# RustAudio/lewton

Hardware: NVIDIA H100
Metric: Msamples/s IMDCT+window+OLA, 2048-pt long blocks (higher is better)
Workload: dtype f32

## Files before the change

### lewton_b200/build.py

```python
import os
import re
import shutil
import subprocess

HERE = os.path.dirname(os.path.abspath(__file__))
CSRC = os.path.join(HERE, "csrc")
SO = os.path.join(HERE, "liblewton_b200.so")
K_LONG_REGS = 249
SOURCES = ["lwb_api.cu", "host_objects.cuh", "path_generic.cuh", "path_long.cuh", "path_chain.cuh", "path_mixed.cuh", "path_mid.cuh",
           "tables_host.cpp", "frontend.cpp", "batcher_submit.cpp", "batcher.h", "lwb_common.h", "pcm_copy_plan.h", "kernels_generic.cuh", "kernel_long.cuh", "kernel_deal.cuh", "kernel_short.cuh", "kernel_mid.cuh", "kernel_chain.cuh", "kernel_prologue.cuh", "kernel_floor0.cuh", "floor1_eval.cuh",
           "floor1_inverse_db.inc", "Makefile"]


def _stale():
    if not os.path.exists(SO):
        return True
    t = os.path.getmtime(SO)
    deps = [os.path.join(CSRC, s) for s in SOURCES] + [os.path.join(HERE, "..", "include", h)
                                                       for h in ("lewton_b200.h", "lewton_frontend.h")]
    return any(os.path.getmtime(d) > t for d in deps)


def check_no_fma(so=SO):
    if shutil.which("cuobjdump") is None:
# ... 41 lines not shown
```

### lewton_b200/csrc/host_objects.cuh

```cuda
#pragma once

struct DevBuf {
    void *p = nullptr;
    size_t cap = 0;
};

struct Staging {
    void *h = nullptr;
    size_t cap = 0;
    cudaEvent_t ev = nullptr;
    bool pending = false;
};

struct ArenaSet {
    DevBuf coeffs, dense, pcm, kinds, ys, vqoff, vqrec;
    cudaEvent_t done = nullptr;
};
constexpr int kHostSets = 2;

struct CachedTables {
    DevTables dt;
    std::vector<float> a, b, c, w;
    std::vector<uint32_t> br;
    std::vector<void *> allocs;
// ... 6 lines not shown
    cudaStream_t copy_in = nullptr, copy_out = nullptr;
    cudaEvent_t ev_in[64] = {}, ev_done[65] = {};
    DevBuf runs_buf[2];
    cudaEvent_t ev_desc[2] = {}, ev_kdone[2] = {};
    int runs_par = 0;
    uint32_t ticket_next = 0;
    uint64_t epoch = 0;
    uint64_t state_gen = 1;
    std::string err;
    uint64_t launches = 0;
    uint64_t kernel_launches[LWB_KERNEL_COUNT] = {};
    std::vector<PcmSpan> pcm_spans;
    std::vector<PcmCopy> pcm_copies;
    std::deque<CachedTables> tables;
    DevBuf spec, segtab, magic, x, desc, chains, ticket, cdesc, cbytes;
    DevBuf floor0;
    ArenaSet host_sets[kHostSets];
    int host_next = 0;
    ArenaSet ordered;
    Staging stage[3];
    int stage_next = 0;
    std::vector<void *> stage_old;
    uint64_t tickets_issued = 0, tickets_done = 0;
    std::deque<cudaEvent_t> ticket_events;
    std::vector<cudaEvent_t> spare_events;
    size_t x_cap_elems = (size_t)64 << 20;
};

struct lwb_setup {
    lwb_ctx *ctx = nullptr;
    DevSetup host;
    DevSetup *d_setup = nullptr;
    std::vector<void *> allocs;
    uint8_t channels = 0, bs0 = 0, bs1 = 0;
    uint32_t n_modes = 0;
    uint32_t n_mappings = 0;
    std::vector<DevMapping> mappings;
    std::vector<uint8_t> floor_types;
    std::vector<DevFloor0> floor0;
    mutable bool streams_opened = false;
    bool floor0_described(uint32_t fi) const { return fi < floor0.size() && floor0[fi].order != 0; }
    unsigned out_channels() const { return host.n_out ? host.n_out : channels; }
};

struct RowCopy { const float *src; float *dst; uint32_t n4, pad; };
struct ChainShape { unsigned warps; size_t smem; int n1max, wpc, np; };

struct Step {
    int kernel;
    const void *desc;
    size_t n;
    const float *pack;
};

struct StepArgs {
    void *pcm = nullptr;
    int out_format = LWB_OUT_F32_PLANAR;
    const float *w_short = nullptr;
    int ls = 0;
    int mid_kb = 0;
// ... 28 lines not shown
    lwb_batch_io io;
    bool captured = false;
    uint64_t gen = 0;
    FrontStages front;
    DevBuf pro, mix;
    StepArgs args;
    std::vector<Step> steps;
};

struct lwb_stream {
    lwb_ctx *ctx = nullptr;
    const lwb_setup *setup = nullptr;
    float *d_state = nullptr;
    bool has = false;
    uint32_t plen = 0;
    uint64_t busy_epoch = 0;
};

static void capture(lwb_plan *plan, uint64_t gen, const FrontStages &front, const StepArgs &args, std::vector<Step> steps)
{
    plan->captured = true;
    plan->gen = gen;
    plan->front = front;
    for (size_t i = 0; i < plan->n_chains && front.n; i++)
        if (!plan->chains[i].stream->setup->floor0.empty()) plan->front.floor0 = true;
    plan->args = args;
    plan->steps = std::move(steps);
}


static inline void set_stream_state(lwb_stream *s, bool has, uint32_t plen)
{
    if (s->has != has || s->plen != plen) {
        s->has = has;
        s->plen = plen;
        s->ctx->state_gen++;
    }
}

static int fail(lwb_ctx *ctx, int code, const char *what, cudaError_t e = cudaSuccess)
{
    if (ctx) {
        ctx->err = what;
        if (e != cudaSuccess) {
            ctx->err += ": ";
            ctx->err += cudaGetErrorString(e);
        }
    }
    return code;
}
// ... 190 lines not shown
```

### lewton_b200/csrc/kernel_long.cuh

```cuda
#pragma once
#include <stdint.h>

#include "lwb_common.h"

#if defined(__CUDACC__)
#include <cuda_fp16.h>
#include <cuda_runtime.h>

#include <type_traits>
#define LWB_HD __host__ __device__ __forceinline__
#else
#define LWB_HD inline
#endif

namespace lwb {

constexpr int kLongBs = 11;
constexpr int kLongN = 2048;
constexpr int kLongN2 = 1024;

struct alignas(16) LongRun {
    const float *in;
    void *out;
    float *state;
    uint32_t in_stride;
    uint32_t n_packets;
    uint8_t has_prev;
    uint8_t write_state;
    uint8_t dummy;
    uint8_t first_short;
    uint8_t last_short;
    uint8_t pad[3];
    float *state_out;
};
static_assert(sizeof(LongRun) == 48, "LongRun is copied by TMA in 16-byte units");

struct V { float x, y; };

#if defined(__CUDA_ARCH__)
__device__ __forceinline__ V vadd(V a, V b) { return V{__fadd_rn(a.x, b.x), __fadd_rn(a.y, b.y)}; }
__device__ __forceinline__ V vsub(V a, V b) { return V{__fsub_rn(a.x, b.x), __fsub_rn(a.y, b.y)}; }
__device__ __forceinline__ V vmul(V a, V b) { return V{__fmul_rn(a.x, b.x), __fmul_rn(a.y, b.y)}; }
__device__ __forceinline__ V vadd_p(V a, V b) { return V{__fadd_rn(a.x, b.x), __fadd_rn(a.y, b.y)}; }
__device__ __forceinline__ V vsub_p(V a, V b) { return V{__fsub_rn(a.x, b.x), __fsub_rn(a.y, b.y)}; }
__device__ __forceinline__ V vnsub_p(V a, V b) { return V{__fsub_rn(-a.x, b.x), __fsub_rn(-a.y, b.y)}; }
#else
inline V vadd(V a, V b) { return V{a.x + b.x, a.y + b.y}; }
// ... 403 lines not shown
#define LWB_KA(j) (4u * (uint32_t)swz(64 * (j)))
#define LWB_KB(j, h) (4u * (uint32_t)swz(((h) << 6) | ((j) << 3)))
#define LWB_KC(j) (4u * (uint32_t)swz(j))

struct RunCur {
    const float *in;
    void *out;
    float *state;
    uint32_t in_stride;
    uint32_t flags;
};
__device__ __forceinline__ RunCur run_cur(const LongRun &r)
{
    return RunCur{r.in, r.out, r.state, r.in_stride,
                  (uint32_t)(r.has_prev ? 1u : 0u) | (r.write_state ? 2u : 0u) | (r.dummy ? 4u : 0u) |
                      (r.first_short ? 8u : 0u) | (r.last_short ? 16u : 0u)};
}
struct RunCurS : RunCur { float *state_out; };
__device__ __forceinline__ RunCurS run_cur_s(const LongRun &r)
{
    RunCurS c;
    static_cast<RunCur &>(c) = run_cur(r);
    c.flags |= r.first_short == 2 ? 32u : 0u;
    c.state_out = r.state_out ? r.state_out : r.state;
    return c;
}

__device__ __forceinline__ int16_t d_sample_i16(float v)
{
    short r;
    asm("cvt.rzi.s16.f32 %0, %1;" : "=h"(r) : "f"(__fmul_rn(v, 32768.0f)));
// ... 12 lines not shown
__device__ __forceinline__ void st_pcm(int16_t *p, float v) { __stcs(reinterpret_cast<short *>(p), (short)d_sample_i16(v)); }
__device__ __forceinline__ void st_pcm(__half *p, float v) { __stcs(reinterpret_cast<short *>(p), __half_as_short(d_sample_f16(v))); }

template <SampleKind K>
using sample_t = std::conditional_t<K == kSampleF32, float, std::conditional_t<K == kSampleI16, int16_t, __half>>;

template <int FORMAT>
__device__ __forceinline__ void store_sample(void *pcm, uint64_t off, uint64_t stride, unsigned channels, unsigned ch,
                                             uint64_t i, float v)
{
    constexpr OutFormat F = out_format_of(FORMAT);
    using T = sample_t<F.kind>;
    static_cast<T *>(pcm)[off + (F.planar ? (uint64_t)ch * stride + i : i * channels + ch)] = d_sample(v, static_cast<T *>(nullptr));
}

template <int NB, bool FIRST, typename OutT, typename RC = RunCur>
__device__ __forceinline__ void out_stage(const TwMix &tw, int lane, const V O[NB][8], const V E[NB][8], V pe[NB][8],
                                          const RC cur[NB], OutT *out[NB], const float *s_state)
{
#pragma unroll
    for (int j = 0; j < 8; j++) {
        const int r64 = 64 * rev3(j);
        const bool nat = (j & 1);
        const V b0 = tw(P_B0 + j), b1 = tw(P_B1 + j);
        const V wlo = tw(P_WLO + j), whi = tw(P_WHI + j);
#pragma unroll
        for (int b = 0; b < NB; b++) {
            V plo = pe[b][j], phi = pe[b][j];
            bool emit = !(cur[b].flags & 4u);
            if (FIRST) {
                emit = emit && (cur[b].flags & 1u);
                if (cur[b].flags & 1u) {
                    const float *s_lo = s_state + b * kLongN2 + lane, *s_hi = s_state + b * kLongN2 + 63 - lane;
                    const float ax = nat ? s_lo[r64] : s_hi[r64], ay = nat ? s_hi[r64] : s_lo[r64];
                    const float bx = nat ? s_hi[960 - r64] : s_lo[960 - r64];
                    const float by = nat ? s_lo[960 - r64] : s_hi[960 - r64];
                    plo = V{ax, ay};
                    phi = V{bx, by};
                }
            }
            V lo, hi, pev;
            step8_ola(b0, b1, wlo, whi, O[b][j], E[b][j], plo, phi, lo, hi, pev);
            pe[b][j] = pev;
            if (emit) {
                OutT *o_lo = out[b] + lane, *o_hi = out[b] + 63 - lane;
                if (nat) {
                    st_pcm(o_lo + r64, lo.x); st_pcm(o_hi + r64, lo.y);
                    st_pcm(o_hi + 960 - r64, hi.x); st_pcm(o_lo + 960 - r64, hi.y);
                } else {
                    st_pcm(o_hi + r64, lo.x); st_pcm(o_lo + r64, lo.y);
                    st_pcm(o_lo + 960 - r64, hi.x); st_pcm(o_hi + 960 - r64, hi.y);
                }
            }
// ... 113 lines not shown
        const uint32_t bar = bars_s + 8 * stage;
        mbar_expect_tx(bar, kLongStageBytes);
#pragma unroll
        for (int b = 0; b < NB; b++)
            tma_load_1d(tiles_s + stage * kLongStageBytes + b * kLongTileBytes,
                        r[b].in + (size_t)pkt * r[b].in_stride, kLongTileBytes, bar);
    };
    auto issue_stage_cur = [&](uint32_t stage, uint32_t pkt) {
        const uint32_t bar = bars_s + 8 * stage;
        mbar_expect_tx(bar, kLongStageBytes);
#pragma unroll
        for (int b = 0; b < NB; b++)
            tma_load_1d(tiles_s + stage * kLongStageBytes + b * kLongTileBytes,
                        cur[b].in + (size_t)pkt * cur[b].in_stride, kLongTileBytes, bar);
    };
    auto issue_state = [&](const float *const st[NB], const uint32_t has[NB]) {
        uint32_t bytes = 0;
#pragma unroll
        for (int b = 0; b < NB; b++) bytes += has[b] ? kLongTileBytes : 0;
        mbar_expect_tx(bar_state, bytes);
#pragma unroll
        for (int b = 0; b < NB; b++)
            if (has[b]) tma_load_1d(state_s + b * kLongTileBytes, st[b], kLongTileBytes, bar_state);
    };

    {
        uint32_t idx = 0;
        if (lane == 0) idx = atomicAdd(ticket, 1u);
        idx = __shfl_sync(0xffffffffu, idx, 0);
        if (idx >= n_groups) return;
#pragma unroll
        for (int b = 0; b < NB; b++) cur[b] = run_cur(runs[idx * NB + b]);
        npk = runs[idx * NB].n_packets;
        if (lane == 0) {
            fence_proxy_async();
            const float *st[NB];
            uint32_t has[NB];
#pragma unroll
            for (int b = 0; b < NB; b++) { st[b] = cur[b].state; has[b] = cur[b].flags & 1u; }
            issue_state(st, has);
            for (; lc < (uint32_t)kLongRing && lc < npk; lc++) issue_stage_cur(lc, lc);
            nx_idx = atomicAdd(ticket, 1u);
        }
    }

    for (;;) {
        V pe[NB][8];
#pragma unroll
        for (int b = 0; b < NB; b++)
#pragma unroll
            for (int j = 0; j < 8; j++) pe[b][j] = V{0.f, 0.f};
        OutT *out[NB];
#pragma unroll
        for (int b = 0; b < NB; b++) out[b] = static_cast<OutT *>(cur[b].out);

// ... 85 lines not shown
                            issue_stage(tgt, s_next, nx_lc);
                            nx_lc++;
                        }
                    }
                }
            }
            phase_c_fft<NB>(tw, O, E);
            if (p > 0) {
                out_stage<NB, false, OutT>(tw, lane, O, E, pe, cur, out, s_state);
            } else {
                mbar_wait(bar_state, (phase_bits >> 30) & 1u);
                phase_bits ^= 1u << 30;
                if (NB == 1 && (cur[0].flags & 8u))
                    out_first_short<NB, OutT>(tw, lane, O, E, pe, cur, out, s_state, w_short, ls);
                else
                    out_stage<NB, true, OutT>(tw, lane, O, E, pe, cur, out, s_state);
                __syncwarp();
            }
#pragma unroll
            for (int b = 0; b < NB; b++)
                if (p > 0 || (cur[b].flags & 1u)) out[b] += (p == 0 && (cur[b].flags & 8u)) ? kLongN2 - ls : kLongN2;
            if (lane == 0 && nx_stage == 2 && !nx_state_issued) {
                const float *st[NB];
                uint32_t has[NB];
#pragma unroll
                for (int b = 0; b < NB; b++) { st[b] = s_next[b].state; has[b] = s_next[b].has_prev; }
                fence_proxy_async();
                issue_state(st, has);
                nx_state_issued = 1;
            }
            slot_i = (slot_i + 1 == (uint32_t)kLongRing) ? 0 : slot_i + 1;
        }
#pragma unroll
        for (int b = 0; b < NB; b++) {
            if ((cur[b].flags & 16u)) {
                const bool emitted = (npk > 1 || (cur[b].flags & 1u)) && !(cur[b].flags & 4u);
                const bool keep = (cur[b].flags & 6u) == 2u;
#pragma unroll
                for (int j = 0; j < 8; j++) {
                    const int r64 = 64 * rev3(j);
#pragma unroll
                    for (int h = 0; h < 2; h++) {
                        const float v = ((j & 1) != 0) == (h == 0) ? pe[b][j].x : pe[b][j].y;
// ... 1 lines not shown
                        if (m < ls) {
                            if (emitted) st_pcm(out[b] + m, v);
                        } else if (keep && m < kLongN2 - ls) {
                            cur[b].state[m - ls] = v;
                            cur[b].state[kLongN2 - 1 - ls - m] = v;
                        }
                    }
                }
            } else if ((cur[b].flags & 6u) == 2u) {
                float *s_lo = cur[b].state + lane, *s_hi = cur[b].state + 63 - lane;
#pragma unroll
                for (int j = 0; j < 8; j++) {
                    const int r64 = 64 * rev3(j);
                    const float vx = (j & 1) ? pe[b][j].x : pe[b][j].y, vy = (j & 1) ? pe[b][j].y : pe[b][j].x;
                    s_lo[r64] = vx; s_hi[r64] = vy;
                    s_hi[960 - r64] = vx; s_lo[960 - r64] = vy;
                }
            }
        }
        uint32_t st_ = 0, nlc = 0;
        if (lane == 0) {
            if (nx_stage == 0) {
                if (nx_idx < n_groups) {
                    fence_proxy_async();
                    mbar_expect_tx(bar_desc, NB * (uint32_t)sizeof(LongRun));
                    tma_load_1d(next_s, runs + (size_t)nx_idx * NB, NB * (uint32_t)sizeof(LongRun), bar_desc);
                    nx_stage = 1;
                } else {
                    nx_stage = 3;
                }
            }
            if (nx_stage == 1) {
                mbar_wait(bar_desc, desc_parity);
                desc_parity ^= 1u;
                nx_stage = 2;
                nx_npk = s_next[0].n_packets;
                nx_lc = 0;
            }
            if (nx_stage == 2 && !nx_state_issued) {
                const float *st[NB];
                uint32_t has[NB];
#pragma unroll
                for (int b = 0; b < NB; b++) { st[b] = s_next[b].state; has[b] = s_next[b].has_prev; }
                fence_proxy_async();
                issue_state(st, has);
            }
            st_ = nx_stage;
            nlc = nx_lc;
        }
        st_ = __shfl_sync(0xffffffffu, st_, 0);
        nlc = __shfl_sync(0xffffffffu, nlc, 0);
        if (st_ != 2) break;
        __syncwarp();
#pragma unroll
        for (int b = 0; b < NB; b++) cur[b] = run_cur(s_next[b]);
        npk = s_next[0].n_packets;
        __syncwarp();
        lc = nlc;
        nx_stage = 0; nx_lc = 0; nx_npk = 0; nx_state_issued = 0;
        if (lane == 0) {
// ... 244 lines not shown
```

### lewton_b200/csrc/lwb_api.cu

```cuda
#include <cuda_runtime.h>
#include <sched.h>
#include <sys/syscall.h>
#include <unistd.h>

#include <algorithm>
#include <cctype>
#include <cmath>
#include <cstdio>
#include <cstdlib>
#include <cstring>
#include <deque>
#include <new>
#include <string>
#include <vector>

#include "kernel_long.cuh"
#include "kernel_short.cuh"
#include "kernel_mid.cuh"
#include "kernels_generic.cuh"
#include "kernel_chain.cuh"
#include "kernel_prologue.cuh"
#include "kernel_floor0.cuh"
#include "lwb_common.h"
#include "pcm_copy_plan.h"
// ... 65 lines not shown
{
    cudaError_t e = cudaStreamSynchronize(ctx->stream);
    for (cudaStream_t s : {ctx->copy_in, ctx->copy_out}) {
        const cudaError_t e2 = s ? cudaStreamSynchronize(s) : cudaSuccess;
        if (e == cudaSuccess) e = e2;
    }
    return e;
}

extern "C" void lwb_ctx_destroy(lwb_ctx *ctx)
{
    if (!ctx) return;
    cudaSetDevice(ctx->device);
    sync_all_streams(ctx);
    for (DevBuf *b : {&ctx->spec, &ctx->segtab, &ctx->magic, &ctx->x, &ctx->desc, &ctx->chains, &ctx->ticket, &ctx->runs_buf[0],
                      &ctx->runs_buf[1], &ctx->cdesc, &ctx->cbytes, &ctx->floor0})
        if (b->p) cudaFree(b->p);
    auto free_set = [](ArenaSet &s) {
        for (DevBuf *b : {&s.coeffs, &s.dense, &s.pcm, &s.kinds, &s.ys, &s.vqoff, &s.vqrec})
            if (b->p) cudaFree(b->p);
        if (s.done) cudaEventDestroy(s.done);
    };
    for (ArenaSet &s : ctx->host_sets) free_set(s);
    free_set(ctx->ordered);
    for (cudaEvent_t e : ctx->ticket_events) cudaEventDestroy(e);
    for (cudaEvent_t e : ctx->spare_events) cudaEventDestroy(e);
    for (CachedTables &ct : ctx->tables)
        for (void *p : ct.allocs) cudaFree(p);
    for (void *h : ctx->stage_old) cudaFreeHost(h);
    for (Staging &st : ctx->stage) {
        if (st.h) cudaFreeHost(st.h);
// ... 432 lines not shown
}

extern "C" void lwb_stream_destroy(lwb_stream *s)
{
    if (!s) return;
    cudaSetDevice(s->ctx->device);
    sync_all_streams(s->ctx);
    cudaFree(s->d_state);
    delete s;
}

extern "C" int lwb_stream_reset(lwb_stream *s)
{
    if (!s) return LWB_ERR_INVALID;
    set_stream_state(s, false, 0);
    return LWB_OK;
}
extern "C" int lwb_stream_is_empty(const lwb_stream *s) { return (!s || !s->has) ? 1 : 0; }
extern "C" uint32_t lwb_stream_state_len(const lwb_stream *s) { return (s && s->has) ? s->plen : 0; }

extern "C" int lwb_stream_clone(const lwb_stream *s, lwb_stream **out)
{
    if (!s || !out) return LWB_ERR_INVALID;
    int rc = lwb_stream_open(s->ctx, s->setup, out);
    if (rc) return rc;
    (*out)->has = s->has;
    (*out)->plen = s->plen;
    lwb_ctx *ctx = s->ctx;
    CU(ctx, cudaMemcpyAsync((*out)->d_state, s->d_state,
                            s->setup->channels * state_stride(s->setup) * sizeof(float),
                            cudaMemcpyDeviceToDevice, ctx->stream));
    return LWB_OK;
}

extern "C" int lwb_stream_export_state(lwb_stream *s, float *out)
{
    if (!s || !out) return LWB_ERR_INVALID;
    if (!s->has) return LWB_OK;
    lwb_ctx *ctx = s->ctx;
    CU(ctx, cudaSetDevice(ctx->device));
    CU(ctx, cudaMemcpy2DAsync(out, s->plen * sizeof(float), s->d_state, state_stride(s->setup) * sizeof(float),
                              s->plen * sizeof(float), s->setup->channels, cudaMemcpyDeviceToHost, ctx->stream));
    CU(ctx, cudaStreamSynchronize(ctx->stream));
    return LWB_OK;
}

extern "C" int lwb_stream_import_state(lwb_stream *s, const float *data, uint32_t len)
{
    if (!s || (!data && len)) return LWB_ERR_INVALID;
    if (len > state_stride(s->setup)) return LWB_ERR_BUFFER;
    lwb_ctx *ctx = s->ctx;
    CU(ctx, cudaSetDevice(ctx->device));
    if (len) {
        CU(ctx, cudaMemcpy2DAsync(s->d_state, state_stride(s->setup) * sizeof(float), data, len * sizeof(float),
                                  len * sizeof(float), s->setup->channels, cudaMemcpyHostToDevice, ctx->stream));
        CU(ctx, cudaStreamSynchronize(ctx->stream));
    }
    s->ctx->state_gen++;
    s->has = true;
    s->plen = len;
    return LWB_OK;
}

extern "C" int lwb_decoded_sample_count(const lwb_setup *su, uint8_t mode, int prev_flag, int next_flag,
                                        uint32_t *n_samples)
{
    if (!su || !n_samples) return LWB_ERR_INVALID;
    Geom g;
    int rc = geometry(su, mode, prev_flag, next_flag, &g);
    if (rc) return rc;
    *n_samples = g.rs - g.ls;
    return LWB_OK;
}

#include "path_generic.cuh"
#include "path_long.cuh"
#include "path_chain.cuh"
#include "path_mixed.cuh"
#include "path_mid.cuh"

using BatchPath = int (*)(lwb_ctx *, const lwb_chain *, size_t, const lwb_batch_io *, const BatchWalk &, bool *, lwb_plan *);
static constexpr BatchPath kBatchPaths[] = {try_long, try_mid, try_mixed, try_chain, try_generic};
constexpr size_t kChainPath = 3, kGenericPath = 4;
static_assert(kBatchPaths[kChainPath] == try_chain && kBatchPaths[kGenericPath] == try_generic && std::size(kBatchPaths) == kGenericPath + 1,
              "kChainPath / kGenericPath name the chain-kernel and the four-kernel path, the last one");

static size_t first_batch_path()
{
    const char *fg = getenv("LWB_FORCE_GENERIC");
    if (!fg) return 0;
    return std::strcmp(fg, "1") == 0 ? kGenericPath : kChainPath;
}

static int check_batch_args(lwb_ctx *ctx, const lwb_chain *chains, size_t n_chains, const lwb_batch_io *io)
{
    if (io->entry != LWB_ENTRY_SPECTRUM && io->entry != LWB_ENTRY_RESIDUE && io->entry != LWB_ENTRY_VQ) return fail(ctx, LWB_ERR_INVALID, "bad entry");
    if (io->memory != LWB_MEM_HOST && io->memory != LWB_MEM_DEVICE) return fail(ctx, LWB_ERR_INVALID, "bad memory space");
    if (!out_format_known(io->out_format)) return fail(ctx, LWB_ERR_INVALID, "bad out_format");
    if (n_chains == 0) return LWB_OK;
    if ((!io->coeffs && io->entry != LWB_ENTRY_VQ) || !io->pcm) return fail(ctx, LWB_ERR_INVALID, "null arena");
// ... 25 lines not shown
    for (size_t i = 0; i < n_chains; i++) {
        const lwb_chain *c = &chains[i];
        const ChainWalk &w = bw->walks[i] = walk_chain(c, [](uint32_t, const Geom &, bool, uint32_t, uint64_t, uint64_t) {});
        if (!w.done) continue;
        if (planar && c->out_stride < w.n_samples) return fail(ctx, LWB_ERR_BUFFER, "chain: out_stride smaller than the samples produced");
        ext.add(io, c, w);
        if (io->entry != LWB_ENTRY_SPECTRUM && (rc = scan_floor_kinds(ctx, io, c, w.done, &ext.need_dense, &ext.need_floor0))) return rc;
    }
    if (ext.need_dense && !io->dense_floor) return fail(ctx, LWB_ERR_INVALID, "dense_floor missing");
    if ((rc = check_vq_offsets(ctx, io, ext.r_lo, ext.r_hi))) return rc;
    if (!pinned_only || io->memory != LWB_MEM_HOST || ext.empty()) return LWB_OK;
    CU(ctx, cudaSetDevice(ctx->device));
    return check_page_locked(ctx, io, ext, chains[0].stream->setup->channels);
}

static int queue_batch(lwb_ctx *ctx, lwb_chain *chains, size_t n_chains, const lwb_batch_io *io, lwb_plan *prepared, bool pinned_only)
{
    if (!ctx || (!chains && n_chains) || !io) return LWB_ERR_INVALID;
    BatchWalk bw;
    int rc = walk_batch(ctx, chains, n_chains, io, pinned_only, &bw);
    if (rc || n_chains == 0) return rc;
    CU(ctx, cudaSetDevice(ctx->device));
    if (prepared) prepared->captured = false;
    size_t first = first_batch_path();
    for (size_t i = 0; i < n_chains && first < kChainPath; i++)
        if (chains[i].stream->setup->host.n_out) first = kChainPath;
    for (size_t k = first; k < std::size(kBatchPaths); k++) {
        bool handled = false;
        if ((rc = kBatchPaths[k](ctx, chains, n_chains, io, bw, &handled, prepared))) return rc;
        if (!handled) continue;
        for (size_t i = 0; i < n_chains; i++) set_chain_result(&chains[i], bw.walks[i]);
        commit_stream_states(chains, bw.walks);
        return LWB_OK;
    }
    return fail(ctx, LWB_ERR_INVALID, "internal: no batch path took the batch");
}

static int decode_chains_impl(lwb_ctx *ctx, lwb_chain *chains, size_t n_chains, const lwb_batch_io *io, lwb_plan *prepared,
                              uint64_t *ticket = nullptr)
{
    if (!ctx) return LWB_ERR_INVALID;
    const uint64_t issued = ctx->tickets_issued;
    int rc = queue_batch(ctx, chains, n_chains, io, prepared, ticket != nullptr);
    if (rc) return rc;
    if (!ticket) return ctx->tickets_issued != issued ? retire_tickets(ctx, ctx->tickets_issued, true) : LWB_OK;
    if (ctx->tickets_issued == issued) {
        CU(ctx, cudaSetDevice(ctx->device));
// ... 119 lines not shown

extern "C" int lwb_decode_packet(lwb_stream *s, const lwb_packet *pkt, int out_format, void *out, size_t cap,
                                 size_t *n_samples)
{
    if (!pkt || !pkt->floor_kind || !pkt->residue) return LWB_ERR_INVALID;
    return one_packet(s, LWB_ENTRY_RESIDUE, pkt->mode_number, pkt->prev_window_flag, pkt->next_window_flag,
                      pkt->residue, pkt, out_format, out, cap, n_samples);
}

extern "C" int lwb_decode_spectrum(lwb_stream *s, uint8_t mode, int prev_flag, int next_flag, const float *spectrum,
                                   int out_format, void *out, size_t cap, size_t *n_samples)
{
    return one_packet(s, LWB_ENTRY_SPECTRUM, mode, prev_flag, next_flag, spectrum, nullptr, out_format, out, cap,
                      n_samples);
}

extern "C" int lwb_debug_packet_taps(lwb_stream *s, const lwb_packet *pkt, float *post_inverse, float *pre_mdct,
                                     float *post_mdct)
{
    if (!s || !pkt || !pkt->floor_kind || !pkt->residue) return LWB_ERR_INVALID;
    lwb_ctx *ctx = s->ctx;
    const lwb_setup *su = s->setup;
    Geom g;
    int rc = geometry(su, pkt->mode_number, pkt->prev_window_flag, pkt->next_window_flag, &g);
    if (rc) return rc;
    CU(ctx, cudaSetDevice(ctx->device));
    const size_t C = su->channels, n2 = g.n >> 1;
    bool need_dense = false, need_y = false, need_floor0 = false;
    for (size_t c = 0; c < C; c++) {
        const uint8_t kd = pkt->floor_kind[c];
// ... 70 lines not shown
```

### lewton_b200/csrc/path_chain.cuh

```cuda
#pragma once

static size_t chain_smem(unsigned maxc, int n1max, int np, bool vq = false)
{
    return (size_t)maxc * ((size_t)np * n1max + n1max / 2) * 4 + 8 * (LWB_MAX_POSTS + 1) * 2 * 2 + 64 +
           (vq ? (size_t)maxc * (n1max / 2) * 4 : 0);
}
static int chain_np(unsigned maxc, int n1max, int wpc, bool residue)
{
    if (residue || wpc != 1) return 1;
    int np = 4;
    while (np > 1 && chain_smem(maxc, n1max, np) > 64 * 1024) np >>= 1;
    return np;
}
static ChainShape chain_shape(unsigned maxc, int n1max, bool residue, bool vq = false)
{
    int wpc = std::max(1, std::min(8, n1max / 1024));
    while (wpc > 1 && (unsigned)wpc * maxc > 32) wpc >>= 1;
    const int np = chain_np(maxc, n1max, wpc, residue);
    return ChainShape{maxc * wpc, chain_smem(maxc, n1max, np, vq), n1max, wpc, np};
}

__global__ void k_row_copy(const RowCopy *__restrict__ rc)
{
    const RowCopy c = rc[blockIdx.x];
    for (uint32_t i = threadIdx.x; i < c.n4; i += blockDim.x)
        reinterpret_cast<float4 *>(c.dst)[i] = reinterpret_cast<const float4 *>(c.src)[i];
}

static void chain_desc(const lwb_chain *c, uint32_t p0, uint32_t n, bool has, uint32_t plen, uint64_t coeff, uint64_t pos, uint32_t byte_off,
                       ChainDesc *d)
{
    const lwb_stream *s = c->stream;
    const lwb_setup *su = s->setup;
    std::memset(d, 0, sizeof(*d));
    d->setup = su->d_setup;
    d->state = s->d_state;
    d->coeff_off = coeff;
    d->out_off = c->out_offset + pos;
    d->out_stride = c->out_stride;
    d->pkt_index = c->packet_index + p0;
    d->n_packets = n;
// ... 99 lines not shown
```

### lewton_b200/csrc/path_generic.cuh

```cuda
#pragma once

struct ChainWalk {
    uint32_t done = 0;
    int status = LWB_OK;
    uint64_t n_samples = 0;
    bool end_has = false;
    uint32_t end_plen = 0;
    bool clear_after = false;
    uint64_t coeff_end = 0;
    uint32_t full_n = 0;
    bool long_only = true;
};

template <typename F>
static ChainWalk walk_chain(const lwb_chain *c, F &&on_packet)
{
    const lwb_setup *su = c->stream->setup;
    ChainWalk w;
    bool has = c->stream->has;
    uint32_t plen = c->stream->plen;
    uint64_t coeff = c->coeff_offset, pos = 0;
    for (uint32_t k = 0; k < c->n_packets; k++) {
        const int pf = c->prev_window_flags ? c->prev_window_flags[k] : 1, nf = c->next_window_flags ? c->next_window_flags[k] : 1;
        Geom g;
// ... 22 lines not shown
    }
    w.n_samples = pos;
    w.end_has = !w.clear_after && has;
    w.end_plen = w.clear_after ? 0 : plen;
    w.coeff_end = coeff;
    return w;
}

static void set_chain_result(lwb_chain *c, const ChainWalk &w)
{
    c->status = w.status;
    c->packets_done = w.done;
    c->n_samples = (uint32_t)w.n_samples;
}

static void commit_stream_states(const lwb_chain *chains, const std::vector<ChainWalk> &walks)
{
    for (size_t i = 0; i < walks.size(); i++)
        if (walks[i].done || walks[i].clear_after) set_stream_state(chains[i].stream, walks[i].end_has, walks[i].end_plen);
}

static void write_mode_bytes(const lwb_chain *c, uint32_t k, uint8_t *out)
{
    out[0] = c->mode_numbers[k];
    out[1] = c->prev_window_flags ? c->prev_window_flags[k] : 1;
    out[2] = c->next_window_flags ? c->next_window_flags[k] : 1;
}

template <typename K, typename... Args>
static int launch(lwb_ctx *ctx, int kernel_id, K kernel, dim3 grid, dim3 block, size_t smem, Args... args)
{
    kernel<<<grid, block, smem, ctx->stream>>>(args...);
    count_launch(ctx, kernel_id);
    cudaError_t e = cudaGetLastError();
// ... 672 lines not shown
```

### lewton_b200/csrc/path_long.cuh

```cuda
#pragma once

struct LongItem {
    const lwb_chain *c;
    uint32_t P;
    bool has_prev;
};

template <typename Run>
static void cut_run(const Run &whole, size_t cuts, size_t first_emit, size_t n2, size_t esz, Run *w)
{
    const size_t P = whole.n_packets;
    for (size_t k = 0; k < cuts; k++) {
        const size_t p0 = P * k / cuts, p1 = P * (k + 1) / cuts;
        Run &r = w[k];
        std::memset(&r, 0, sizeof(r));
        r.in_stride = whole.in_stride;
        r.state = whole.state;
        r.write_state = (k + 1 == cuts);
        if (k == 0) {
            r.in = whole.in;
            r.out = whole.out;
            r.n_packets = (uint32_t)(p1 - p0);
            r.has_prev = whole.has_prev;
        } else {
// ... 6 lines not shown
    }
}

template <typename Run>
static void channel_run(const lwb_chain *c, unsigned ch, size_t n2, const float *in, char *pcm, size_t esz, uint32_t n, bool has,
                        size_t first_emit, size_t cuts, Run *w)
{
    const lwb_stream *s = c->stream;
    const lwb_setup *su = s->setup;
    const unsigned C = su->channels;
    cut_run(Run{in + (size_t)ch * n2, pcm + (c->out_offset + (size_t)ch * c->out_stride) * esz, s->d_state + (size_t)ch * state_stride(su),
                (uint32_t)(C * n2), n, has},
            cuts, first_emit, n2, esz, w);
}

static void long_runs_of(const LongItem &it, size_t cuts, const float *coeffs, char *pcm, size_t esz, LongRun *&w)
{
    for (unsigned ch = 0; ch < it.c->stream->setup->channels; ch++, w += cuts)
        channel_run(it.c, ch, kLongN2, coeffs + it.c->coeff_offset, pcm, esz, it.P, it.has_prev, it.has_prev ? kLongN2 : 0, cuts, w);
}

static bool batch_is_uniform_long(const lwb_chain *chains, size_t n_chains, const lwb_batch_io *io, const BatchWalk &bw)
{
    if (!fused_layout(chains, n_chains, io)) return false;
    const float *pack = nullptr;
    for (size_t i = 0; i < n_chains; i++) {
        const lwb_chain *c = &chains[i];
        const lwb_stream *s = c->stream;
        const lwb_setup *su = s->setup;
        if (su->bs1 != kLongBs || !su->host.tab[1].pack) return false;
        if (pack && pack != su->host.tab[1].pack) return false;
        pack = su->host.tab[1].pack;
        if (s->has && s->plen != (uint32_t)kLongN2) return false;
        if (bw.walks[i].done != c->n_packets || !bw.walks[i].long_only) return false;
    }
    return true;
}

struct LongRuns {
    struct Chunk { size_t r0, nr; };
    std::vector<Chunk> chunks;
    Staging *st = nullptr;
    LongRun *h = nullptr, *d = nullptr;
    size_t n = 0;
    int par = 0;
    bool own = false;
};

static int long_build_runs(lwb_ctx *ctx, const lwb_chain *chains, size_t n_chains, size_t n_chunks, const float *coeffs, char *pcm,
                           size_t esz, DevBuf *own, LongRuns *lr)
{
    std::vector<LongItem> items;
    items.reserve(n_chains);
    size_t chan_chains = 0;
    for (size_t i = 0; i < n_chains; i++) {
        const lwb_chain *c = &chains[i];
        items.push_back(LongItem{c, c->n_packets, c->stream->has});
        if (c->n_packets) chan_chains += c->stream->setup->channels;
    }
    const size_t warp_slots = (size_t)ctx->sm_count * kLongWarps * kLongNB;
    size_t target_runs = warp_slots * 4;
    if (const char *e = getenv("LWB_LONG_TARGET_RUNS")) target_runs = (size_t)atol(e);
    const size_t min_run = 8;
    int rc;
    std::vector<size_t> cuts(items.size(), 1);
// ... 18 lines not shown
    lr->h = h_runs;
    std::vector<LongRun> tmp;
    std::vector<uint32_t> order;
    for (size_t k = 0; k < n_chunks; k++) {
        const size_t i0 = items.size() * k / n_chunks, i1 = items.size() * (k + 1) / n_chunks;
        LongRun *w0 = w;
        size_t chunk_runs = 0;
        for (size_t i = i0; i < i1; i++)
            if (items[i].P) chunk_runs += cuts[i] * items[i].c->stream->setup->channels;
        LongRun *gen = w;
        if (kLongNB > 1) {
            tmp.resize(chunk_runs);
            gen = tmp.data();
        }
        for (size_t i = i0; i < i1; i++)
            if (items[i].P) long_runs_of(items[i], cuts[i], coeffs, pcm, esz, gen);
        if (kLongNB == 1) {
            w = gen;
        } else {
            bool sorted = true;
            for (size_t i = 1; i < tmp.size() && sorted; i++) sorted = tmp[i].n_packets == tmp[0].n_packets;
            order.resize(tmp.size());
            for (uint32_t i = 0; i < order.size(); i++) order[i] = i;
            if (!sorted)
                std::stable_sort(order.begin(), order.end(),
                                 [&](uint32_t a, uint32_t b) { return tmp[a].n_packets < tmp[b].n_packets; });
            size_t i = 0;
            while (i < order.size()) {
                size_t j = i;
                while (j < order.size() && tmp[order[j]].n_packets == tmp[order[i]].n_packets) j++;
                for (size_t q = i; q < j; q++) *w++ = tmp[order[q]];
// ... 13 lines not shown
    lr->n = (size_t)(w - h_runs);
    return LWB_OK;
}

static int long_upload_runs(lwb_ctx *ctx, const LongRuns &lr, cudaStream_t ds)
{
    int rc;
    if (lr.own && ds != ctx->stream && (rc = order_copies_behind_compute(ctx))) return rc;
    CU(ctx, cudaStreamWaitEvent(ds, ctx->ev_kdone[lr.par], 0));
    if ((rc = upload_staging(ctx, lr.st, lr.h, lr.d, lr.n * sizeof(LongRun), ds))) return rc;
    CU(ctx, cudaEventRecord(ctx->ev_desc[lr.par], ds));
    CU(ctx, cudaStreamWaitEvent(ctx->stream, ctx->ev_desc[lr.par], 0));
    return LWB_OK;
}

static int try_long(lwb_ctx *ctx, const lwb_chain *chains, size_t n_chains, const lwb_batch_io *io, const BatchWalk &bw, bool *handled,
                    lwb_plan *plan)
{
    *handled = false;
    if (!batch_is_uniform_long(chains, n_chains, io, bw)) return LWB_OK;
    *handled = true;
    const BatchExtent &ext = bw.ext;
    if (ext.empty()) return LWB_OK;
    int rc;
    const unsigned C = chains[0].stream->setup->channels;
    const bool residue = io->entry != LWB_ENTRY_SPECTRUM, host = io->memory == LWB_MEM_HOST;
    const float *pack = chains[0].stream->setup->host.tab[1].pack;
    const size_t n_chunks = host ? host_chunks((size_t)(ext.c_hi - ext.c_lo) * 4, n_chains) : 1;
    const bool cap = plan && !host;
    BatchArenas ar;
// ... 17 lines not shown
    StepArgs args;
    args.pcm = ar.pcm;
    args.out_format = io->out_format;
    std::vector<Step> steps;
    LongRuns lr;
    uint64_t gen = 0;
    size_t pk0 = 0;
    for (size_t k = 0; k < n_chunks; k++) {
        const size_t i0 = n_chains * k / n_chunks, i1 = n_chains * (k + 1) / n_chunks;
        const BatchExtent ke = chunk_extent(io, chains, bw, i0, i1);
        if (ke.empty()) continue;
        size_t npk = 0;
        for (size_t i = i0; i < i1; i++) npk += chains[i].n_packets;
        if ((rc = ar.upload(k, ke)) || (residue && (rc = front_stages_launch(ctx, ar, fs, pk0, npk)))) return rc;
        if (!lr.d) {
            if ((rc = long_build_runs(ctx, chains, n_chains, n_chunks, in, ar.pcm, out_format_of(io->out_format).esz, cap ? &plan->mix : nullptr, &lr)) ||
                (rc = long_upload_runs(ctx, lr, host ? ctx->copy_in : ctx->copy_out)))
                return rc;
            gen = ctx->state_gen;
        }
        steps.assign(1, Step{LWB_KERNEL_LONG, lr.d + lr.chunks[k].r0, lr.chunks[k].nr / kLongNB, pack});
        if ((rc = run_steps(ctx, args, steps)) || (rc = ar.download(k, chains, bw, i0, i1, ke))) return rc;
        pk0 += npk;
    }
    CU(ctx, cudaEventRecord(ctx->ev_kdone[lr.par], ctx->stream));
    if (cap) capture(plan, gen, fs, args, std::move(steps));
    return ar.finish();
}
```

Before: 316,900.

## Store long-block overlap state as mirrored half rows

The long-block kernel now writes only half of each overlap-add state row when the run ends a captured plan, because the saved tail is symmetric. It then loads only half a tile through TMA at the start of the next batch and rebuilds the other half in registers. Streams carry a mirror flag, so other batch paths and host readback unfold the half rows on demand, either with a mirrored row-copy kernel or on the host. The aim is to cut state memory traffic. The cost is extra bookkeeping, an extra unfold launch when a stream switches paths, and slightly higher register use.

New measurement: 324,700 (median of 6 runs). 2.5% higher.

```diff
diff --git a/lewton_b200/build.py b/lewton_b200/build.py
--- a/lewton_b200/build.py
+++ b/lewton_b200/build.py
@@ -6,7 +6,7 @@
 HERE = os.path.dirname(os.path.abspath(__file__))
 CSRC = os.path.join(HERE, "csrc")
 SO = os.path.join(HERE, "liblewton_b200.so")
-K_LONG_REGS = 249
+K_LONG_REGS = 251
 SOURCES = ["lwb_api.cu", "host_objects.cuh", "path_generic.cuh", "path_long.cuh", "path_chain.cuh", "path_mixed.cuh", "path_mid.cuh",
            "tables_host.cpp", "frontend.cpp", "batcher_submit.cpp", "batcher.h", "lwb_common.h", "pcm_copy_plan.h", "kernels_generic.cuh", "kernel_long.cuh", "kernel_deal.cuh", "kernel_short.cuh", "kernel_mid.cuh", "kernel_chain.cuh", "kernel_prologue.cuh", "kernel_floor0.cuh", "floor1_eval.cuh",
            "floor1_inverse_db.inc", "Makefile"]
diff --git a/lewton_b200/csrc/host_objects.cuh b/lewton_b200/csrc/host_objects.cuh
--- a/lewton_b200/csrc/host_objects.cuh
+++ b/lewton_b200/csrc/host_objects.cuh
@@ -44,6 +44,7 @@
     std::vector<PcmCopy> pcm_copies;
     std::deque<CachedTables> tables;
     DevBuf spec, segtab, magic, x, desc, chains, ticket, cdesc, cbytes;
+    DevBuf unfold;
     DevBuf floor0;
     ArenaSet host_sets[kHostSets];
     int host_next = 0;
@@ -73,7 +74,7 @@
     unsigned out_channels() const { return host.n_out ? host.n_out : channels; }
 };
 
-struct RowCopy { const float *src; float *dst; uint32_t n4, pad; };
+struct RowCopy { const float *src; float *dst; uint32_t n4, mirror; };
 struct ChainShape { unsigned warps; size_t smem; int n1max, wpc, np; };
 
 struct Step {
@@ -132,6 +133,7 @@
     float *d_state = nullptr;
     bool has = false;
     uint32_t plen = 0;
+    bool mirror = false;
     uint64_t busy_epoch = 0;
 };
 
@@ -152,6 +154,14 @@
     if (s->has != has || s->plen != plen) {
         s->has = has;
         s->plen = plen;
+        s->ctx->state_gen++;
+    }
+}
+
+static inline void set_stream_mirror(lwb_stream *s, bool mirror)
+{
+    if (s->mirror != mirror) {
+        s->mirror = mirror;
         s->ctx->state_gen++;
     }
 }
diff --git a/lewton_b200/csrc/kernel_long.cuh b/lewton_b200/csrc/kernel_long.cuh
--- a/lewton_b200/csrc/kernel_long.cuh
+++ b/lewton_b200/csrc/kernel_long.cuh
@@ -30,7 +30,9 @@
     uint8_t dummy;
     uint8_t first_short;
     uint8_t last_short;
-    uint8_t pad[3];
+    uint8_t mirror_in;
+    uint8_t mirror_out;
+    uint8_t pad;
     float *state_out;
 };
 static_assert(sizeof(LongRun) == 48, "LongRun is copied by TMA in 16-byte units");
@@ -464,7 +466,8 @@
 {
     return RunCur{r.in, r.out, r.state, r.in_stride,
                   (uint32_t)(r.has_prev ? 1u : 0u) | (r.write_state ? 2u : 0u) | (r.dummy ? 4u : 0u) |
-                      (r.first_short ? 8u : 0u) | (r.last_short ? 16u : 0u)};
+                      (r.first_short ? 8u : 0u) | (r.last_short ? 16u : 0u) | (r.mirror_in ? 64u : 0u) |
+                      (r.mirror_out ? 128u : 0u)};
 }
 struct RunCurS : RunCur { float *state_out; };
 __device__ __forceinline__ RunCurS run_cur_s(const LongRun &r)
@@ -507,7 +510,7 @@
     static_cast<T *>(pcm)[off + (F.planar ? (uint64_t)ch * stride + i : i * channels + ch)] = d_sample(v, static_cast<T *>(nullptr));
 }
 
-template <int NB, bool FIRST, typename OutT, typename RC = RunCur>
+template <int NB, bool FIRST, typename OutT, typename RC = RunCur, bool MIRROR = false>
 __device__ __forceinline__ void out_stage(const TwMix &tw, int lane, const V O[NB][8], const V E[NB][8], V pe[NB][8],
                                           const RC cur[NB], OutT *out[NB], const float *s_state)
 {
@@ -526,10 +529,14 @@
                 if (cur[b].flags & 1u) {
                     const float *s_lo = s_state + b * kLongN2 + lane, *s_hi = s_state + b * kLongN2 + 63 - lane;
                     const float ax = nat ? s_lo[r64] : s_hi[r64], ay = nat ? s_hi[r64] : s_lo[r64];
-                    const float bx = nat ? s_hi[960 - r64] : s_lo[960 - r64];
-                    const float by = nat ? s_lo[960 - r64] : s_hi[960 - r64];
                     plo = V{ax, ay};
-                    phi = V{bx, by};
+                    if (MIRROR && (cur[b].flags & 64u)) {
+                        phi = plo;
+                    } else {
+                        const float bx = nat ? s_hi[960 - r64] : s_lo[960 - r64];
+                        const float by = nat ? s_lo[960 - r64] : s_hi[960 - r64];
+                        phi = V{bx, by};
+                    }
                 }
             }
             V lo, hi, pev;
@@ -673,15 +680,16 @@
             tma_load_1d(tiles_s + stage * kLongStageBytes + b * kLongTileBytes,
                         cur[b].in + (size_t)pkt * cur[b].in_stride, kLongTileBytes, bar);
     };
-    auto issue_state = [&](const float *const st[NB], const uint32_t has[NB]) {
+    auto issue_state = [&](const float *const st[NB], const uint32_t len[NB]) {
         uint32_t bytes = 0;
 #pragma unroll
-        for (int b = 0; b < NB; b++) bytes += has[b] ? kLongTileBytes : 0;
+        for (int b = 0; b < NB; b++) bytes += len[b];
         mbar_expect_tx(bar_state, bytes);
 #pragma unroll
         for (int b = 0; b < NB; b++)
-            if (has[b]) tma_load_1d(state_s + b * kLongTileBytes, st[b], kLongTileBytes, bar_state);
+            if (len[b]) tma_load_1d(state_s + b * kLongTileBytes, st[b], len[b], bar_state);
     };
+    auto state_len = [](bool has, bool mirror) -> uint32_t { return has ? (mirror ? kLongTileBytes / 2 : kLongTileBytes) : 0; };
 
     {
         uint32_t idx = 0;
@@ -694,10 +702,10 @@
         if (lane == 0) {
             fence_proxy_async();
             const float *st[NB];
-            uint32_t has[NB];
-#pragma unroll
-            for (int b = 0; b < NB; b++) { st[b] = cur[b].state; has[b] = cur[b].flags & 1u; }
-            issue_state(st, has);
+            uint32_t len[NB];
+#pragma unroll
+            for (int b = 0; b < NB; b++) { st[b] = cur[b].state; len[b] = state_len(cur[b].flags & 1u, cur[b].flags & 64u); }
+            issue_state(st, len);
             for (; lc < (uint32_t)kLongRing && lc < npk; lc++) issue_stage_cur(lc, lc);
             nx_idx = atomicAdd(ticket, 1u);
         }
@@ -813,7 +821,7 @@
                 if (NB == 1 && (cur[0].flags & 8u))
                     out_first_short<NB, OutT>(tw, lane, O, E, pe, cur, out, s_state, w_short, ls);
                 else
-                    out_stage<NB, true, OutT>(tw, lane, O, E, pe, cur, out, s_state);
+                    out_stage<NB, true, OutT, RunCur, true>(tw, lane, O, E, pe, cur, out, s_state);
                 __syncwarp();
             }
 #pragma unroll
@@ -821,11 +829,11 @@
                 if (p > 0 || (cur[b].flags & 1u)) out[b] += (p == 0 && (cur[b].flags & 8u)) ? kLongN2 - ls : kLongN2;
             if (lane == 0 && nx_stage == 2 && !nx_state_issued) {
                 const float *st[NB];
-                uint32_t has[NB];
-#pragma unroll
-                for (int b = 0; b < NB; b++) { st[b] = s_next[b].state; has[b] = s_next[b].has_prev; }
+                uint32_t len[NB];
+#pragma unroll
+                for (int b = 0; b < NB; b++) { st[b] = s_next[b].state; len[b] = state_len(s_next[b].has_prev, s_next[b].mirror_in); }
                 fence_proxy_async();
-                issue_state(st, has);
+                issue_state(st, len);
                 nx_state_issued = 1;
             }
             slot_i = (slot_i + 1 == (uint32_t)kLongRing) ? 0 : slot_i + 1;
@@ -857,7 +865,9 @@
                     const int r64 = 64 * rev3(j);
                     const float vx = (j & 1) ? pe[b][j].x : pe[b][j].y, vy = (j & 1) ? pe[b][j].y : pe[b][j].x;
                     s_lo[r64] = vx; s_hi[r64] = vy;
-                    s_hi[960 - r64] = vx; s_lo[960 - r64] = vy;
+                    if (!(cur[b].flags & 128u)) {
+                        s_hi[960 - r64] = vx; s_lo[960 - r64] = vy;
+                    }
                 }
             }
         }
@@ -882,11 +892,11 @@
             }
             if (nx_stage == 2 && !nx_state_issued) {
                 const float *st[NB];
-                uint32_t has[NB];
-#pragma unroll
-                for (int b = 0; b < NB; b++) { st[b] = s_next[b].state; has[b] = s_next[b].has_prev; }
+                uint32_t len[NB];
+#pragma unroll
+                for (int b = 0; b < NB; b++) { st[b] = s_next[b].state; len[b] = state_len(s_next[b].has_prev, s_next[b].mirror_in); }
                 fence_proxy_async();
-                issue_state(st, has);
+                issue_state(st, len);
             }
             st_ = nx_stage;
             nlc = nx_lc;
diff --git a/lewton_b200/csrc/lwb_api.cu b/lewton_b200/csrc/lwb_api.cu
--- a/lewton_b200/csrc/lwb_api.cu
+++ b/lewton_b200/csrc/lwb_api.cu
@@ -103,7 +103,7 @@
     cudaSetDevice(ctx->device);
     sync_all_streams(ctx);
     for (DevBuf *b : {&ctx->spec, &ctx->segtab, &ctx->magic, &ctx->x, &ctx->desc, &ctx->chains, &ctx->ticket, &ctx->runs_buf[0],
-                      &ctx->runs_buf[1], &ctx->cdesc, &ctx->cbytes, &ctx->floor0})
+                      &ctx->runs_buf[1], &ctx->cdesc, &ctx->cbytes, &ctx->floor0, &ctx->unfold})
         if (b->p) cudaFree(b->p);
     auto free_set = [](ArenaSet &s) {
         for (DevBuf *b : {&s.coeffs, &s.dense, &s.pcm, &s.kinds, &s.ys, &s.vqoff, &s.vqrec})
@@ -566,6 +566,7 @@
 {
     if (!s) return LWB_ERR_INVALID;
     set_stream_state(s, false, 0);
+    set_stream_mirror(s, false);
     return LWB_OK;
 }
 extern "C" int lwb_stream_is_empty(const lwb_stream *s) { return (!s || !s->has) ? 1 : 0; }
@@ -578,6 +579,7 @@
     if (rc) return rc;
     (*out)->has = s->has;
     (*out)->plen = s->plen;
+    (*out)->mirror = s->mirror;
     lwb_ctx *ctx = s->ctx;
     CU(ctx, cudaMemcpyAsync((*out)->d_state, s->d_state,
                             s->setup->channels * state_stride(s->setup) * sizeof(float),
@@ -591,9 +593,14 @@
     if (!s->has) return LWB_OK;
     lwb_ctx *ctx = s->ctx;
     CU(ctx, cudaSetDevice(ctx->device));
+    const uint32_t n = s->mirror ? s->plen / 2 : s->plen;
     CU(ctx, cudaMemcpy2DAsync(out, s->plen * sizeof(float), s->d_state, state_stride(s->setup) * sizeof(float),
-                              s->plen * sizeof(float), s->setup->channels, cudaMemcpyDeviceToHost, ctx->stream));
+                              n * sizeof(float), s->setup->channels, cudaMemcpyDeviceToHost, ctx->stream));
     CU(ctx, cudaStreamSynchronize(ctx->stream));
+    for (unsigned ch = 0; ch < s->setup->channels && s->mirror; ch++) {
+        float *row = out + (size_t)ch * s->plen;
+        for (uint32_t m = 0; m < n; m++) row[s->plen - 1 - m] = row[m];
+    }
     return LWB_OK;
 }
 
@@ -611,6 +618,7 @@
     s->ctx->state_gen++;
     s->has = true;
     s->plen = len;
+    s->mirror = false;
     return LWB_OK;
 }
 
@@ -633,9 +641,10 @@
 
 using BatchPath = int (*)(lwb_ctx *, const lwb_chain *, size_t, const lwb_batch_io *, const BatchWalk &, bool *, lwb_plan *);
 static constexpr BatchPath kBatchPaths[] = {try_long, try_mid, try_mixed, try_chain, try_generic};
-constexpr size_t kChainPath = 3, kGenericPath = 4;
-static_assert(kBatchPaths[kChainPath] == try_chain && kBatchPaths[kGenericPath] == try_generic && std::size(kBatchPaths) == kGenericPath + 1,
-              "kChainPath / kGenericPath name the chain-kernel and the four-kernel path, the last one");
+constexpr size_t kLongPath = 0, kChainPath = 3, kGenericPath = 4;
+static_assert(kBatchPaths[kLongPath] == try_long && kBatchPaths[kChainPath] == try_chain && kBatchPaths[kGenericPath] == try_generic &&
+                  std::size(kBatchPaths) == kGenericPath + 1,
+              "kLongPath / kChainPath / kGenericPath name the all-long, the chain-kernel and the four-kernel path, the last one");
 
 static size_t first_batch_path()
 {
@@ -691,6 +700,29 @@
     return check_page_locked(ctx, io, ext, chains[0].stream->setup->channels);
 }
 
+static int unfold_mirror_rows(lwb_ctx *ctx, const lwb_chain *chains, size_t n_chains, const std::vector<ChainWalk> &walks)
+{
+    size_t n = 0;
+    for (size_t i = 0; i < n_chains; i++)
+        if (chains[i].stream->mirror && walks[i].done) n += chains[i].stream->setup->channels;
+    if (!n) return LWB_OK;
+    int rc;
+    Staging *st;
+    if ((rc = acquire_staging(ctx, n * sizeof(RowCopy), &st)) || (rc = ensure(ctx, ctx->unfold, n * sizeof(RowCopy)))) return rc;
+    RowCopy *h = (RowCopy *)st->h, *w = h;
+    for (size_t i = 0; i < n_chains; i++) {
+        lwb_stream *s = chains[i].stream;
+        if (!s->mirror || !walks[i].done) continue;
+        for (unsigned ch = 0; ch < s->setup->channels; ch++) {
+            float *row = s->d_state + (size_t)ch * state_stride(s->setup);
+            *w++ = RowCopy{row, row, (uint32_t)(s->plen / 8), 1};
+        }
+        set_stream_mirror(s, false);
+    }
+    if ((rc = upload_staging(ctx, st, h, ctx->unfold.p, n * sizeof(RowCopy), ctx->stream))) return rc;
+    return launch(ctx, LWB_KERNEL_ROW_COPY, k_row_copy, dim3((unsigned)n), dim3(64), 0, (const RowCopy *)ctx->unfold.p);
+}
+
 static int queue_batch(lwb_ctx *ctx, lwb_chain *chains, size_t n_chains, const lwb_batch_io *io, lwb_plan *prepared, bool pinned_only)
 {
     if (!ctx || (!chains && n_chains) || !io) return LWB_ERR_INVALID;
@@ -704,10 +736,11 @@
         if (chains[i].stream->setup->host.n_out) first = kChainPath;
     for (size_t k = first; k < std::size(kBatchPaths); k++) {
         bool handled = false;
+        if (k != kLongPath && (rc = unfold_mirror_rows(ctx, chains, n_chains, bw.walks))) return rc;
         if ((rc = kBatchPaths[k](ctx, chains, n_chains, io, bw, &handled, prepared))) return rc;
         if (!handled) continue;
         for (size_t i = 0; i < n_chains; i++) set_chain_result(&chains[i], bw.walks[i]);
-        commit_stream_states(chains, bw.walks);
+        commit_stream_states(chains, bw.walks, k == kLongPath && leaves_mirror_halves(prepared));
         return LWB_OK;
     }
     return fail(ctx, LWB_ERR_INVALID, "internal: no batch path took the batch");
@@ -857,6 +890,8 @@
     return one_packet(s, LWB_ENTRY_SPECTRUM, mode, prev_flag, next_flag, spectrum, nullptr, out_format, out, cap,
                       n_samples);
 }
+
+extern "C" int lwb_debug_stream_mirror(const lwb_stream *s) { return s && s->mirror ? 1 : 0; }
 
 extern "C" int lwb_debug_packet_taps(lwb_stream *s, const lwb_packet *pkt, float *post_inverse, float *pre_mdct,
                                      float *post_mdct)
diff --git a/lewton_b200/csrc/path_chain.cuh b/lewton_b200/csrc/path_chain.cuh
--- a/lewton_b200/csrc/path_chain.cuh
+++ b/lewton_b200/csrc/path_chain.cuh
@@ -23,8 +23,11 @@
 __global__ void k_row_copy(const RowCopy *__restrict__ rc)
 {
     const RowCopy c = rc[blockIdx.x];
-    for (uint32_t i = threadIdx.x; i < c.n4; i += blockDim.x)
-        reinterpret_cast<float4 *>(c.dst)[i] = reinterpret_cast<const float4 *>(c.src)[i];
+    for (uint32_t i = threadIdx.x; i < c.n4; i += blockDim.x) {
+        const float4 v = reinterpret_cast<const float4 *>(c.src)[i];
+        if (c.mirror) reinterpret_cast<float4 *>(c.dst)[2 * c.n4 - 1 - i] = make_float4(v.w, v.z, v.y, v.x);
+        else reinterpret_cast<float4 *>(c.dst)[i] = v;
+    }
 }
 
 static void chain_desc(const lwb_chain *c, uint32_t p0, uint32_t n, bool has, uint32_t plen, uint64_t coeff, uint64_t pos, uint32_t byte_off,
diff --git a/lewton_b200/csrc/path_generic.cuh b/lewton_b200/csrc/path_generic.cuh
--- a/lewton_b200/csrc/path_generic.cuh
+++ b/lewton_b200/csrc/path_generic.cuh
@@ -60,10 +60,13 @@
     c->n_samples = (uint32_t)w.n_samples;
 }
 
-static void commit_stream_states(const lwb_chain *chains, const std::vector<ChainWalk> &walks)
+static void commit_stream_states(const lwb_chain *chains, const std::vector<ChainWalk> &walks, bool halves)
 {
     for (size_t i = 0; i < walks.size(); i++)
-        if (walks[i].done || walks[i].clear_after) set_stream_state(chains[i].stream, walks[i].end_has, walks[i].end_plen);
+        if (walks[i].done || walks[i].clear_after) {
+            set_stream_state(chains[i].stream, walks[i].end_has, walks[i].end_plen);
+            set_stream_mirror(chains[i].stream, halves && walks[i].end_has);
+        }
 }
 
 static void write_mode_bytes(const lwb_chain *c, uint32_t k, uint8_t *out)
diff --git a/lewton_b200/csrc/path_long.cuh b/lewton_b200/csrc/path_long.cuh
--- a/lewton_b200/csrc/path_long.cuh
+++ b/lewton_b200/csrc/path_long.cuh
@@ -44,10 +44,13 @@
             cuts, first_emit, n2, esz, w);
 }
 
-static void long_runs_of(const LongItem &it, size_t cuts, const float *coeffs, char *pcm, size_t esz, LongRun *&w)
-{
-    for (unsigned ch = 0; ch < it.c->stream->setup->channels; ch++, w += cuts)
+static void long_runs_of(const LongItem &it, size_t cuts, const float *coeffs, char *pcm, size_t esz, bool halves, LongRun *&w)
+{
+    for (unsigned ch = 0; ch < it.c->stream->setup->channels; ch++, w += cuts) {
         channel_run(it.c, ch, kLongN2, coeffs + it.c->coeff_offset, pcm, esz, it.P, it.has_prev, it.has_prev ? kLongN2 : 0, cuts, w);
+        w[0].mirror_in = it.has_prev && it.c->stream->mirror;
+        w[cuts - 1].mirror_out = halves;
+    }
 }
 
 static bool batch_is_uniform_long(const lwb_chain *chains, size_t n_chains, const lwb_batch_io *io, const BatchWalk &bw)
@@ -78,7 +81,7 @@
 };
 
 static int long_build_runs(lwb_ctx *ctx, const lwb_chain *chains, size_t n_chains, size_t n_chunks, const float *coeffs, char *pcm,
-                           size_t esz, DevBuf *own, LongRuns *lr)
+                           size_t esz, bool halves, DevBuf *own, LongRuns *lr)
 {
     std::vector<LongItem> items;
     items.reserve(n_chains);
@@ -127,7 +130,7 @@
             gen = tmp.data();
         }
         for (size_t i = i0; i < i1; i++)
-            if (items[i].P) long_runs_of(items[i], cuts[i], coeffs, pcm, esz, gen);
+            if (items[i].P) long_runs_of(items[i], cuts[i], coeffs, pcm, esz, halves, gen);
         if (kLongNB == 1) {
             w = gen;
         } else {
@@ -171,6 +174,8 @@
     return LWB_OK;
 }
 
+static bool leaves_mirror_halves(const lwb_plan *plan) { return plan != nullptr; }
+
 static int try_long(lwb_ctx *ctx, const lwb_chain *chains, size_t n_chains, const lwb_batch_io *io, const BatchWalk &bw, bool *handled,
                     lwb_plan *plan)
 {
@@ -218,7 +223,8 @@
         for (size_t i = i0; i < i1; i++) npk += chains[i].n_packets;
         if ((rc = ar.upload(k, ke)) || (residue && (rc = front_stages_launch(ctx, ar, fs, pk0, npk)))) return rc;
         if (!lr.d) {
-            if ((rc = long_build_runs(ctx, chains, n_chains, n_chunks, in, ar.pcm, out_format_of(io->out_format).esz, cap ? &plan->mix : nullptr, &lr)) ||
+            if ((rc = long_build_runs(ctx, chains, n_chains, n_chunks, in, ar.pcm, out_format_of(io->out_format).esz, leaves_mirror_halves(plan),
+                                      cap ? &plan->mix : nullptr, &lr)) ||
                 (rc = long_upload_runs(ctx, lr, host ? ctx->copy_in : ctx->copy_out)))
                 return rc;
             gen = ctx->state_gen;
diff --git a/profiles/long_state_bytes.py b/profiles/long_state_bytes.py
--- /dev/null
+++ b/profiles/long_state_bytes.py
@@ -0,0 +1,100 @@
+import argparse
+import ctypes as C
+import json
+import os
+import subprocess
+import sys
+
+import numpy as np
+
+sys.path.insert(0, os.path.dirname(os.path.dirname(os.path.abspath(__file__))))
+
+import lewton_b200 as L
+from lewton_b200 import _cabi as cabi
+
+N2 = 1024
+
+
+def gpu_info():
+    import torch
+    name = torch.cuda.get_device_name(0)
+    try:
+        q = subprocess.run(["nvidia-smi", "--query-gpu=power.limit,clocks.sm,clocks.max.sm", "--format=csv,noheader", "-i", "0"],
+                           capture_output=True, text=True, timeout=30).stdout.strip()
+    except (OSError, subprocess.SubprocessError):
+        q = "unknown"
+    return name, q
+
+
+def mirror_query():
+    f = getattr(cabi.lib(), "lwb_debug_stream_mirror", None)
+    if f is not None:
+        f.restype, f.argtypes = C.c_int, [C.c_void_p]
+    return f
+
+
+def one_shape(ctx, su, stream, S, P, steps, warmup):
+    import torch
+    Ch = 2
+    stride = P * N2
+    gen = torch.Generator(device="cuda").manual_seed(1234)
+    spec = torch.randn((S, P, Ch, N2), generator=gen, device="cuda", dtype=torch.float32) * 1e-2
+    pcm = torch.empty((S, Ch, stride), device="cuda", dtype=torch.float32)
+    torch.cuda.synchronize()
+    pwrs = [L.PreviousWindowRight(su) for _ in range(S)]
+    modes = np.ones(P, np.uint8)
+    chains = [L.ChainSpec(pwrs[s], modes, coeff_offset=s * P * Ch * N2, out_offset=s * Ch * stride, out_stride=stride)
+              for s in range(S)]
+    batch = L.Batch(ctx, chains, cabi.ENTRY_SPECTRUM, cabi.MEM_DEVICE, spec.data_ptr(), pcm.data_ptr(), cabi.OUT_F32_PLANAR)
+    for _ in range(max(warmup, 3)):
+        batch.run()
+    ctx.synchronize()
+    q = mirror_query()
+    half = bool(q and all(q(p._h) for p in pwrs))
+    k0 = ctx.kernel_launches()
+    e0, e1 = torch.cuda.Event(enable_timing=True), torch.cuda.Event(enable_timing=True)
+    e0.record(stream)
+    for _ in range(steps):
+        batch.run()
+    e1.record(stream)
+    ctx.synchronize()
+    torch.cuda.synchronize()
+    k1 = ctx.kernel_launches()
+    ms = e0.elapsed_time(e1) / steps
+    samples = S * P * Ch * N2
+    row = N2 * 4 // (2 if half else 1)
+    nbytes = samples * 8 + S * Ch * row * 2
+    out = {"P": P, "streams": S, "ms_per_step": ms, "model_bytes": nbytes, "state_row_bytes": row,
+           "gbs": nbytes / (ms * 1e-3) / 1e9, "msamples_per_s": samples / (ms * 1e-3) / 1e6,
+           "launches_per_step": {k: (k1[k] - k0[k]) / steps for k in k1 if k1[k] != k0[k]}}
+    batch.close()
+    for p in pwrs:
+        p.close()
+    del spec, pcm
+    return out
+
+
+def main():
+    import torch
+    ap = argparse.ArgumentParser()
+    ap.add_argument("--total", type=int, default=4096 * 16, help="stream-packets per step (S * P)")
+    ap.add_argument("--packets", default="1,2,4,16,64")
+    ap.add_argument("--steps", type=int, default=20)
+    ap.add_argument("--warmup", type=int, default=5)
+    args = ap.parse_args()
+    ctx = L.Context(0)
+    su = L.Setup(ctx, 2, 8, 11, [L.FloorTypeOne(1, [0, 128])], [L.Mapping(2)], [L.ModeInfo(False), L.ModeInfo(True)])
+    stream = torch.cuda.ExternalStream(ctx.cuda_stream, device=torch.device("cuda", 0))
+    name, q = gpu_info()
+    rows = []
+    for P in (int(x) for x in args.packets.split(",")):
+        r = one_shape(ctx, su, stream, args.total // P, P, args.steps, args.warmup)
+        rows.append(r)
+        print(f"P={P:3d} S={r['streams']:6d}  {r['ms_per_step']:.4f} ms/step  {r['model_bytes'] / 2**20:7.0f} MiB  "
+              f"{r['gbs']:7.1f} GB/s  state row {r['state_row_bytes']} B", file=sys.stderr)
+    ctx.close()
+    print(json.dumps({"gpu": name, "power_limit_sm_clock_max_clock": q, "lib": cabi.SO_PATH, "rows": rows}))
+
+
+if __name__ == "__main__":
+    sys.exit(main())
```
